# xujiabo/SCREAM

Hardware: AMD Instinct MI355X
Metric: registration pairs/sec (higher is better)
Workload: dtype f32; 1 GPU; BASELINE configs[1]: synthetic 3DMatch_test-like pairs, voxel 0.0625 m, ~5k points/cloud, batch-of-pairs=32 per GPU, A1-A10 per pair (forward 6+6 layers d_model 256, 1-NN thresh 0.1, Kabsch, RE/TE), random-init weights seed 0; lanes=1, steps_in_flight=2, parallelism=dp1 (pairs sharded, metric-row all-gather), rccl_ranks=1, gemm_backend=h2

## Files before the change

### include/scream_hip.h

```cpp
#ifndef SCREAM_HIP_H
#define SCREAM_HIP_H

#include <stdint.h>

#ifdef __cplusplus
extern "C" {
#endif

#define SCREAM_ROW_TILE 128
#define SCREAM_D_MODEL 256
#define SCREAM_NHEAD 8
#define SCREAM_HEAD_DIM 32
#define SCREAM_KV_CHUNK 256

#define SCREAM_EINVAL (-1)
#define SCREAM_EUNSUPPORTED (-2)

enum {
    SCREAM_EPI_NONE = 0,
    SCREAM_EPI_ELU1 = 1,
    SCREAM_EPI_RELU = 2,
    SCREAM_EPI_BIAS_RELU = 3,
    SCREAM_EPI_RES_LN = 4,
    SCREAM_EPI_QKV = 5
// ... 28 lines not shown
                          const float* residual, int64_t ldr, const float* gamma, const float* beta,
                          int32_t layout, int32_t split, int32_t a_exp, int32_t w_exp, void* stream);
int scream_gemm_qkv_split_f32(const float* A, int64_t lda, const void* W_packed, float* Q, int64_t ldq,
                              int64_t M, int32_t N, int32_t K, int32_t n_q, const int32_t* tile_cloud,
                              const int32_t* cloud_row0, const int32_t* cloud_len, int64_t row_base,
                              float* kv_partial, int32_t layout, int32_t split, int32_t a_exp, int32_t w_exp,
                              int32_t k_exp, int32_t v_exp, void* stream);

int64_t scream_proj_image_bytes(int32_t N, int32_t split);
int scream_pack_proj(const float* W, int32_t N, int32_t n_q, int32_t split, int32_t w_exp, void* proj_image, void* stream);
int scream_proj_qkv_f32(const float* x, const void* proj_image, float* Q, int64_t M, int32_t N, int32_t n_q,
                        const int32_t* tile_cloud, const int32_t* cloud_row0, const int32_t* cloud_len,
                        int64_t row_base, float* kv_partial, int32_t split, int32_t a_exp, int32_t w_exp, int32_t k_exp,
                        int32_t v_exp, void* stream);

typedef struct {
    int32_t e_att, e_wm, e_m1, e_w1, e_h, e_w2;
    int32_t e_y, e_wq;
    int32_t e_q;
} scream_tail_exps_t;
int64_t scream_tail_image_bytes(int32_t split, int32_t with_next_q);
int64_t scream_kv_image_bytes(void);
int scream_pack_tail(const float* Wm, const float* W1, const float* W2, const float* Wq_next, int32_t split,
                     const scream_tail_exps_t* exps, void* tail_image, void* stream);
int scream_kv_finalize_image(const float* kv_partial, const int32_t* cloud_row0, const int32_t* cloud_len,
                          int64_t row_base, int32_t cloud_begin, int32_t n_kv, void* kv_image, int32_t n_layers,
                          int64_t partial_layer_stride, int64_t image_layer_stride, int32_t split, void* stream);
int scream_layer_tail_f32(const float* Q, const void* kv_image, const int32_t* tile_cloud,
                          int32_t kv_cloud_offset, const int32_t* cloud_len, const float* x,
                          const void* tail_image, const float* g1, const float* b1, const float* g2,
                          const float* b2, float* y, float* q_next, int64_t M, int32_t split,
                          const scream_tail_exps_t* exps, void* stream);

int scream_pe_embed_ln(const float* xyz, const int32_t* tile_cloud, const float* center,
                       const float* dim_t, const float* emb_w, const float* emb_b,
                       const float* gamma, const float* beta, float* feats, int64_t rows,
                       void* stream);
int scream_pe_embed_ln_frag(const float* xyz, const int32_t* tile_cloud, const float* center,
                            const float* dim_t, const float* emb_w, const float* emb_b,
                            const float* gamma, const float* beta, float* feats, int64_t rows,
                            void* stream);

int scream_kv_reduce(const float* Kf, const float* Vf, int64_t ld, int64_t row_base,
                     const int32_t* cloud_row0, const int32_t* cloud_len, int32_t cloud_begin,
                     int32_t n_kv, int32_t max_chunks, float* partial, float* kv_out, void* stream);

int scream_attn_apply(const float* Qf, int64_t ldq, const float* kv, const int32_t* tile_cloud,
                      int32_t kv_cloud_offset, const int32_t* cloud_len, float* out, int64_t ldo,
                      int64_t rows, void* stream);

int scream_coor_head(const float* X, const float* W, const float* b, float* out, int64_t rows,
                     void* stream);

typedef struct {
    const float* wqkv;
    const float* wq;
    const float* wkv;
    const float* wm;
    const float* w1;
    const float* w2;
    const float* g1; const float* b1;
    const float* g2; const float* b2;
    const void* tail;
    int32_t e_xq, e_xkv, e_wqkv, e_wq, e_wkv, e_wm_g, e_w1_g, e_w2_g;
    int32_t e_k, e_v;
    scream_tail_exps_t tail_exps;
    int32_t tail_next_q;
    const void* proj;
} scream_layer_t;

typedef struct {
    int32_t n_self;
    int32_t n_cross;
    const float* dim_t;
    const float* emb_w; const float* emb_b;
    const float* pre_g; const float* pre_b;
    const scream_layer_t* layers_host;
    const float* c0_w; const float* c0_b;
    const float* c2_w; const float* c2_b;
    const float* c4_w; const float* c4_b;
    const scream_layer_t* stem_tgt_layers_host;
    int32_t gemm_split;
    int32_t e_c0x, e_c0w, e_c2x, e_c2w;
    const float* wkv_cross;
    int32_t e_wkv_cross, e_k_cross, e_v_cross;
    const void* proj_cross;
} scream_model_t;

typedef struct {
    int32_t n_pairs;
    int64_t rows_src;
    int64_t rows_total;
    int32_t max_chunks;
    const float* xyz;
    const float* center;
    const int32_t* tile_cloud;
    const int32_t* cloud_row0;
    const int32_t* cloud_len;
} scream_batch_t;

int64_t scream_forward_workspace_bytes(int64_t rows_src, int64_t rows_total, int32_t n_pairs,
                                       int32_t max_chunks, int32_t fused_tail, int32_t n_cross_batched);

int scream_forward(const scream_model_t* model, const scream_batch_t* batch, void* workspace,
                   int64_t workspace_bytes, float* src_pred, float* feats_out, void* trace,
                   void* stream);

void* scream_trace_create(int32_t capacity);
void scream_trace_destroy(void* trace);
int scream_trace_reset(void* trace);
int scream_trace_read(void* trace, int32_t max_records, float* ms, int32_t* kind, int64_t* m,
                      int32_t* n, int32_t* k);
int scream_trace_read_starts(void* trace, int32_t max_records, float* start_ms);

int scream_nn_search(const float* query, const float* ref, const int32_t* q_row0,
                     const int32_t* q_len, const int32_t* r_row0, const int32_t* r_len,
                     const float* s, int32_t n_pairs, int32_t max_q_len, int32_t max_r_len,
                     int64_t q_rows_total, int64_t r_rows_total, float thresh, float* ref_prep,
                     uint64_t* keys, int32_t* idx, float* dmin, uint8_t* valid, void* stream);

int scream_square_distance(const float* src, const float* dst, float* out, int32_t B, int32_t N,
                           int32_t M, void* stream);

int scream_kabsch_corr(const float* src, const float* ref, const int32_t* src_row0,
                       const int32_t* src_len, const int32_t* ref_row0, const int32_t* idx,
                       const uint8_t* valid, const float* s, const float* c, int32_t n_pairs,
                       float* T_out, int32_t* n_corr, void* stream);

int scream_rigid_transform_3d(const float* A, const float* B, const float* w,
                              float weight_threshold, int32_t bs, int32_t K, float* T_out,
                              void* stream);

int scream_transformation_error(const float* T_pred, const float* T_gt, int32_t n, float* re,
                                float* te, void* stream);

int scream_point_loss(const float* src_pred, const float* src, const int32_t* src_row0, const int32_t* src_len,
                      const float* rot, const float* trans, int32_t n_pairs, float* loss, void* stream);

int64_t scream_icp_workspace_bytes(int64_t src_rows_total, int64_t ref_rows_total, int32_t n_pairs);
// ... 65 lines not shown
```

### scream_amd/_lib.py

```python
from __future__ import annotations

import ctypes as C
import os
from typing import Optional

_HERE = os.path.dirname(os.path.abspath(__file__))
LIB_PATH = os.environ.get("SCREAM_LIB") or os.path.join(_HERE, "libscream_hip.so")
ABI_VERSION = 20

c_f32p = C.POINTER(C.c_float)
c_i32p = C.POINTER(C.c_int32)
c_u8p = C.POINTER(C.c_uint8)
c_u64p = C.POINTER(C.c_uint64)


SPLIT_H1, SPLIT_H2, SPLIT_BF3 = 1, 2, 3


class TailExpsT(C.Structure):
    _fields_ = [(n, C.c_int32) for n in ("e_att", "e_wm", "e_m1", "e_w1", "e_h", "e_w2", "e_y", "e_wq", "e_q")]


class LayerT(C.Structure):
    _fields_ = ([(n, C.c_void_p) for n in ("wqkv", "wq", "wkv", "wm", "w1", "w2", "g1", "b1", "g2", "b2", "tail")] +
                [(n, C.c_int32) for n in ("e_xq", "e_xkv", "e_wqkv", "e_wq", "e_wkv", "e_wm_g", "e_w1_g", "e_w2_g", "e_k", "e_v")] +
                [("tail_exps", TailExpsT), ("tail_next_q", C.c_int32), ("proj", C.c_void_p)])


class ModelT(C.Structure):
    _fields_ = [("n_self", C.c_int32), ("n_cross", C.c_int32), ("dim_t", C.c_void_p), ("emb_w", C.c_void_p),
                ("emb_b", C.c_void_p), ("pre_g", C.c_void_p), ("pre_b", C.c_void_p),
                ("layers_host", C.POINTER(LayerT)), ("c0_w", C.c_void_p), ("c0_b", C.c_void_p),
                ("c2_w", C.c_void_p), ("c2_b", C.c_void_p), ("c4_w", C.c_void_p), ("c4_b", C.c_void_p),
                ("stem_tgt_layers_host", C.POINTER(LayerT)), ("gemm_split", C.c_int32),
                ("e_c0x", C.c_int32), ("e_c0w", C.c_int32), ("e_c2x", C.c_int32), ("e_c2w", C.c_int32),
                ("wkv_cross", C.c_void_p), ("e_wkv_cross", C.c_int32), ("e_k_cross", C.c_int32), ("e_v_cross", C.c_int32),
                ("proj_cross", C.c_void_p)]


class BatchT(C.Structure):
    _fields_ = [("n_pairs", C.c_int32), ("rows_src", C.c_int64), ("rows_total", C.c_int64),
                ("max_chunks", C.c_int32), ("xyz", C.c_void_p), ("center", C.c_void_p),
                ("tile_cloud", C.c_void_p), ("cloud_row0", C.c_void_p), ("cloud_len", C.c_void_p)]


V, I32, I64, F32 = C.c_void_p, C.c_int32, C.c_int64, C.c_float
SIGNATURES = {
    "scream_version": (C.c_char_p, []),
    "scream_abi_version": (C.c_int, []),
    "scream_gemm_f32": (C.c_int, [V, I64, V, V, I64, I64, I32, I32, I32, I32, V, V, I64, V, V, V]),
    "scream_gemm_qkv_f32": (C.c_int, [V, I64, V, V, I64, I64, I32, I32, I32, V, V, V, I64, V, V]),
    "scream_kv_finalize": (C.c_int, [V, V, V, I64, I32, I32, V, V]),
    "scream_pack_w_split": (C.c_int, [V, I32, I32, I32, I32, V, V]),
    "scream_gemm_split_f32": (C.c_int, [V, I64, V, V, I64, I64, I32, I32, I32, I32, V, V, I64, V, V, I32, I32, I32, I32, V]),
    "scream_gemm_qkv_split_f32": (C.c_int, [V, I64, V, V, I64, I64, I32, I32, I32, V, V, V, I64, V, I32, I32, I32, I32, I32, I32, V]),
    "scream_proj_image_bytes": (C.c_int64, [I32, I32]),
    "scream_pack_proj": (C.c_int, [V, I32, I32, I32, I32, V, V]),
    "scream_proj_qkv_f32": (C.c_int, [V, V, V, I64, I32, I32, V, V, V, I64, V, I32, I32, I32, I32, I32, V]),
    "scream_tail_image_bytes": (C.c_int64, [I32, I32]),
    "scream_kv_image_bytes": (C.c_int64, []),
    "scream_pack_tail": (C.c_int, [V, V, V, V, I32, C.POINTER(TailExpsT), V, V]),
    "scream_kv_finalize_image": (C.c_int, [V, V, V, I64, I32, I32, V, I32, I64, I64, I32, V]),
    "scream_layer_tail_f32": (C.c_int, [V, V, V, I32, V, V, V, V, V, V, V, V, V, I64, I32, C.POINTER(TailExpsT), V]),
    "scream_act_layout": (C.c_int, [V, V, I64, I32, V]),
    "scream_pe_embed_ln": (C.c_int, [V, V, V, V, V, V, V, V, V, I64, V]),
    "scream_pe_embed_ln_frag": (C.c_int, [V, V, V, V, V, V, V, V, V, I64, V]),
    "scream_kv_reduce": (C.c_int, [V, V, I64, I64, V, V, I32, I32, I32, V, V, V]),
    "scream_attn_apply": (C.c_int, [V, I64, V, V, I32, V, V, I64, I64, V]),
    "scream_coor_head": (C.c_int, [V, V, V, V, I64, V]),
    "scream_forward_workspace_bytes": (C.c_int64, [I64, I64, I32, I32, I32, I32]),
    "scream_forward": (C.c_int, [C.POINTER(ModelT), C.POINTER(BatchT), V, I64, V, V, V, V]),
    "scream_trace_create": (C.c_void_p, [I32]),
    "scream_trace_destroy": (None, [V]),
    "scream_trace_reset": (C.c_int, [V]),
    "scream_trace_read": (C.c_int, [V, I32, V, V, V, V, V]),
    "scream_trace_read_starts": (C.c_int, [V, I32, V]),
    "scream_nn_search": (C.c_int, [V, V, V, V, V, V, V, I32, I32, I32, I64, I64, F32, V, V, V, V, V, V]),
    "scream_square_distance": (C.c_int, [V, V, V, I32, I32, I32, V]),
    "scream_kabsch_corr": (C.c_int, [V, V, V, V, V, V, V, V, V, I32, V, V, V]),
    "scream_rigid_transform_3d": (C.c_int, [V, V, V, F32, I32, I32, V, V]),
    "scream_transformation_error": (C.c_int, [V, V, I32, V, V, V]),
    "scream_point_loss": (C.c_int, [V, V, V, V, V, V, I32, V, V]),
    "scream_icp_workspace_bytes": (C.c_int64, [I64, I64, I32]),
    "scream_icp_p2p": (C.c_int, [V, V, V, V, V, V, V, V, I32, I32, I32, I64, I64, F32, I32, F32, F32, V, V, V, V, I64, V]),
    "scream_wgrad_workspace_bytes": (C.c_int64, [I64, I32, I32]),
    "scream_gemm_wgrad_f32": (C.c_int, [V, I64, V, I64, I64, I32, I32, V, I32, V, V, I64, V]),
    "scream_wgrad_split_workspace_bytes": (C.c_int64, [I64, I32, I32]),
    "scream_gemm_wgrad_split_f32": (C.c_int, [V, I64, V, I64, I64, I32, I32, V, I32, V, I32, V, I64, V]),
    "scream_ln_fwd": (C.c_int, [V, V, V, V, V, V, V, I64, V]),
    "scream_ln_bwd_workspace_bytes": (C.c_int64, [I64]),
    "scream_ln_bwd": (C.c_int, [V, V, V, V, V, V, V, V, V, V, I32, I64, V, I64, V]),
    "scream_attn_bwd_workspace_bytes": (C.c_int64, [I32, I32]),
    "scream_attn_bwd": (C.c_int, [V, I64, I64, I64, V, V, V, V, I64, I64, I64, V, V, V, V, I32, I32, I32, I32, V, I64, V, V, I64,
                                  V, I64, V]),
    "scream_relu_bwd": (C.c_int, [V, V, I64, V]),
    "scream_add_f32": (C.c_int, [V, V, I64, V]),
    "scream_transpose_f32": (C.c_int, [V, I32, I32, V, V]),
    "scream_coor_head_bwd": (C.c_int, [V, V, V, V, I64, V]),
    "scream_grad3_workspace_bytes": (C.c_int64, [I64]),
    "scream_grad3": (C.c_int, [V, V, V, V, I64, V, I32, V, V, I32, V, I64, V]),
    "scream_pe_embed": (C.c_int, [V, V, V, V, V, V, V, I64, V]),
    "scream_icp_p2p_range": (C.c_int, [V, V, V, V, V, V, V, V, I32, I32, I32, I64, I64, F32, I32, F32, F32, V, V, V, I32, I32, V, V, I64, V]),
    "scream_render_workspace_bytes": (C.c_int64, [I32, I32, I32, I64]),
    "scream_render_depth": (C.c_int, [V, V, V, V, V, V, I32, I32, I32, I64, V, I32, I32, F32, V, V, V, I64, V]),
    "scream_render_depth_bwd": (C.c_int, [V, V, V, I32, I32, I64, V, I32, I32, F32, V, V, V, I64, V, V]),
    "scream_voxel_workspace_bytes": (C.c_int64, [I64, I32]),
    "scream_voxel_down_sample": (C.c_int, [V, V, V, I32, I32, V, V, V, V, V, I64, V]),
}

_lib: Optional[C.CDLL] = None


class ScreamHipError(RuntimeError):
    pass


def load() -> C.CDLL:
    global _lib
    if _lib is not None:
        return _lib
    if os.environ.get("SCREAM_NO_BUILD", "0") != "1" and not os.environ.get("SCREAM_LIB"):
        try:
# ... 30 lines not shown
```

### scream_amd/build.py

```python
from __future__ import annotations

import os
import shutil
import subprocess
import sys
from concurrent.futures import ThreadPoolExecutor

HERE = os.path.dirname(os.path.abspath(__file__))
CSRC = os.path.join(HERE, "csrc")
LIB = os.path.join(HERE, "libscream_hip.so")
ARCH = "gfx950"

SOURCES = {
    "gemm_f32.hip": [],
    "gemm_split.hip": [],
    "proj_ring.hip": ["-mllvm", "-amdgpu-mfma-vgpr-form=1"],
    "tail_split.hip": ["-ffp-contract=off"],
    "embed.hip": [],
    "attention.hip": [],
    "backward.hip": [],
    "forward.hip": [],
    "nn_search.hip": ["-ffp-contract=off"],
    "kabsch.hip": ["-ffp-contract=off"],
    "icp_grid.hip": ["-ffp-contract=off"],
    "render.hip": ["-ffp-contract=off"],
    "voxel.hip": ["-ffp-contract=off"],
}
ASM_LOADS = ("gemm_split.hip", "tail_split.hip", "proj_ring.hip")
NO_SCRATCH = {"proj_ring.hip": ("proj_ring_kernel",), "tail_split.hip": ("tail_kernelINS_7SplitH2", "tail_kernelINS_7SplitH1")}


def _hipcc() -> str:
    exe = shutil.which("hipcc") or "/opt/rocm/bin/hipcc"
    if not os.path.exists(exe):
        raise RuntimeError("hipcc not found: cannot build libscream_hip.so")
    return exe


def _stale() -> bool:
    if not os.path.exists(LIB):
        return True
    t = os.path.getmtime(LIB)
    deps = [os.path.join(CSRC, f) for f in os.listdir(CSRC)] + [os.path.join(HERE, "..", "include", "scream_hip.h"), __file__]
    return any(os.path.getmtime(d) > t for d in deps)


def build(force: bool = False, verbose: bool = False, out: str = None) -> str:
    global LIB
    if out:
        LIB, force = out, True
    if not force and not _stale():
        return LIB
    hipcc = _hipcc()
    objdir = os.path.join(HERE, "build")
    os.makedirs(objdir, exist_ok=True)
    common = [hipcc, "-O3", "-std=c++17", "--offload-arch=" + ARCH, "-fPIC", "-Wall", "-Wno-unused-function"]

    def compile_one(item):
        src, extra = item
        obj = os.path.join(objdir, src.replace(".hip", ".o"))
        cmd = common + extra + ["-c", os.path.join(CSRC, src), "-o", obj]
        r = subprocess.run(cmd, capture_output=True, text=True)
        if r.returncode != 0:
            raise RuntimeError("hipcc failed for %s:\n%s\n%s" % (src, " ".join(cmd), r.stderr))
        if verbose and r.stderr.strip():
            print(r.stderr, file=sys.stderr)
        return obj

    def verify_one(src):
        sys.path.insert(0, os.path.join(HERE, "..", "tools"))
        import asm_inflight_check as chk
        asm = os.path.join(objdir, src.replace(".hip", ".s"))
        cmd = common + SOURCES[src] + ["-S", "--cuda-device-only", os.path.join(CSRC, src), "-o", asm]
        r = subprocess.run(cmd, capture_output=True, text=True)
        if r.returncode != 0:
            raise RuntimeError("hipcc -S failed for %s:\n%s" % (src, r.stderr))
        for name, body in chk.kernels(asm):
            if any(k in name for k in NO_SCRATCH.get(src, ())) and any(("scratch_" in l or "buffer_store" in l) for l in body):
                raise RuntimeError("%s: %s spills registers to scratch (this hipcc allocates registers differently from the one the "
                                   "kernel was written with)" % (src, name))
            bad = chk.check_kernel(name, body)
            if bad:
# ... 33 lines not shown
```

### scream_amd/csrc/forward.hip

```cpp
#include <vector>

#include "common.h"

namespace {

constexpr int D = SCREAM_D_MODEL;
constexpr int KV_ELEMS = (SCREAM_HEAD_DIM + 1) * SCREAM_HEAD_DIM;

struct Workspace {
    float *x0, *x1, *q, *att, *m1, *hid, *kvp, *kv;
    char* kvimg;
    float* kvp_cross;
    char* kvimg_cross;
    int64_t kvp_cross_stride, kvimg_cross_stride;
    int64_t bytes;
};

Workspace carve(void* base, int64_t rows_src, int64_t rows_total, int32_t n_pairs, int32_t max_chunks, bool fused, int32_t n_cross_batched) {
    Workspace w;
    float* p = reinterpret_cast<float*>(base);
    auto take = [&](int64_t n) {
        float* r = p;
        p += (n + 63) / 64 * 64;
        return r;
// ... 234 lines not shown
    SCREAM_REQUIRE(m.layers_host && m.n_self >= 0 && m.n_cross >= 0 &&
                       (m.gemm_split == 0 || m.gemm_split == SCREAM_SPLIT_H1 || m.gemm_split == SCREAM_SPLIT_H2 || m.gemm_split == SCREAM_SPLIT_BF3),
                   SCREAM_EINVAL);
    SCREAM_REQUIRE(b.n_pairs > 0 && b.rows_src > 0 && b.rows_total > b.rows_src && b.max_chunks > 0, SCREAM_EINVAL);
    SCREAM_REQUIRE(b.rows_src % SCREAM_ROW_TILE == 0 && b.rows_total % SCREAM_ROW_TILE == 0, SCREAM_EUNSUPPORTED);
    SCREAM_REQUIRE(b.xyz && b.center && b.tile_cloud && b.cloud_row0 && b.cloud_len, SCREAM_EINVAL);
    int n_layers = m.n_self + 2 * m.n_cross, n_tail = 0;
    for (int i = 0; i < n_layers; ++i) n_tail += m.layers_host[i].tail != nullptr;
    if (m.stem_tgt_layers_host)
        for (int i = 0; i < m.n_self; ++i, ++n_layers) n_tail += m.stem_tgt_layers_host[i].tail != nullptr;
    SCREAM_REQUIRE(n_tail == 0 || (n_tail == n_layers && m.gemm_split != 0), SCREAM_EINVAL);
    uintptr_t base = (reinterpret_cast<uintptr_t>(workspace) + 255) & ~(uintptr_t)255;
    const bool batched_kv = n_tail > 0 && m.wkv_cross != nullptr && m.n_cross > 0;
    const Workspace w = carve(reinterpret_cast<void*>(base), b.rows_src, b.rows_total, b.n_pairs, b.max_chunks, n_tail > 0,
                              batched_kv ? m.n_cross : 0);
    SCREAM_REQUIRE((int64_t)(base - reinterpret_cast<uintptr_t>(workspace)) + w.bytes <= workspace_bytes, SCREAM_EINVAL);
    const Ctx c{stream, reinterpret_cast<Trace*>(trace), m.gemm_split, n_tail > 0};

    const int64_t rs = b.rows_src, ra = b.rows_total;
    {
        Scope sc(c.tr, TR_EMBED, ra, 0, 0, stream);
        if (c.frag)
            TRY(scream_pe_embed_ln_frag(b.xyz, b.tile_cloud, b.center, m.dim_t, m.emb_w, m.emb_b, m.pre_g, m.pre_b, w.x0, ra, stream));
        else
            TRY(scream_pe_embed_ln(b.xyz, b.tile_cloud, b.center, m.dim_t, m.emb_w, m.emb_b, m.pre_g, m.pre_b, w.x0, ra, stream));
    }
    float* cur = w.x0;
    float* nxt = w.x1;
    for (int i = 0; i < m.n_self; ++i) {
        if (!m.stem_tgt_layers_host) {
            TRY(mha_self(c, m.layers_host[i], b, w, cur, nxt, 0, ra, 0, 2 * b.n_pairs));
        } else {
            TRY(mha_self(c, m.layers_host[i], b, w, cur, nxt, 0, rs, 0, b.n_pairs));
            TRY(mha_self(c, m.stem_tgt_layers_host[i], b, w, cur, nxt, rs, ra - rs, b.n_pairs, b.n_pairs));
        }
        float* t = cur;
        cur = nxt;
        nxt = t;
    }
    const float* x_tgt = cur + rs * D;
    if (batched_kv) TRY(cross_kv_all(c, m, b, w, x_tgt));
    for (int i = 0; i < 2 * m.n_cross; ++i) {
        const scream_layer_t& L = m.layers_host[m.n_self + i];
        if (i % 2 == 0) {
            TRY(mha_self(c, L, b, w, cur, nxt, 0, rs, 0, b.n_pairs, c.frag && L.tail_next_q));
        } else {
            const bool q_ready = c.frag && m.layers_host[m.n_self + i - 1].tail_next_q;
            TRY(mha_cross(c, L, b, w, cur, x_tgt, nxt, batched_kv ? w.kvimg_cross + (i / 2) * w.kvimg_cross_stride : nullptr, q_ready));
        }
        float* t = cur;
        cur = nxt;
        nxt = t;
    }
    float* c_mid = c.frag ? w.q : w.m1;
    float* c_out = c.frag ? nxt : w.att;
    TRY(gemm(c, cur, D, m.c0_w, c_mid, D, rs, D, D, SCREAM_EPI_BIAS_RELU, 0, m.c0_b, nullptr, nullptr, nullptr, m.e_c0x, m.e_c0w,
             c.frag ? SCREAM_LAYOUT_A_FRAG : 0));
    TRY(gemm(c, c_mid, D, m.c2_w, c_out, D, rs, D, D, SCREAM_EPI_BIAS_RELU, 0, m.c2_b, nullptr, nullptr, nullptr, m.e_c2x, m.e_c2w));
    {
        Scope sc(c.tr, TR_COOR_HEAD, rs, 0, 0, stream);
        TRY(scream_coor_head(c_out, m.c4_w, m.c4_b, src_pred, rs, stream));
    }
    if (feats_out && c.frag) {
        TRY(scream_act_layout(cur, feats_out, rs, 0, stream));
    } else if (feats_out) {
        hipError_t e = hipMemcpyAsync(feats_out, cur, (size_t)rs * D * sizeof(float), hipMemcpyDeviceToDevice,
                                      as_stream(stream));
        if (e != hipSuccess) return (int)e;
    }
    return 0;
}
```

### scream_amd/model.py

```python
from __future__ import annotations

import ctypes as C
import os
from typing import List, Optional, Sequence, Tuple

import torch
from torch import nn

from . import _lib, ops, scales
from .packing import PackedBatch
from .render import RegistrationRender

D_MODEL = 256
NHEAD = 8


class _MHAParams(nn.Module):

    def __init__(self, d_model: int, nhead: int = NHEAD):
        super().__init__()
        self.q_proj = nn.Linear(d_model, d_model, bias=False)
        self.k_proj = nn.Linear(d_model, d_model, bias=False)
        self.v_proj = nn.Linear(d_model, d_model, bias=False)
        self.merge = nn.Linear(d_model, d_model, bias=False)
# ... 33 lines not shown
            raise NotImplementedError("the gfx950 kernels are built for d_model=256 (8 heads x 32), the only "
                                      "configuration the reference evaluates (evaluate_3d_match.py:188)")
        self.embedding = nn.Conv1d(3, d_model, kernel_size=1, stride=1)
        self.pre_norm = nn.LayerNorm(d_model)
        self.self_layer_num = self_layer_num
        self.cross_layer_num = cross_layer_num
        self.stem = nn.ModuleList([_MHAParams(d_model) for _ in range(self_layer_num)])
        self.cross = nn.ModuleList()
        for _ in range(cross_layer_num):
            self.cross.append(_MHAParams(d_model))
            self.cross.append(_CrossParams(d_model))
        self.coor_mlp = nn.Sequential(nn.Conv1d(d_model, d_model, 1), nn.ReLU(), nn.Conv1d(d_model, d_model, 1),
                                      nn.ReLU(), nn.Conv1d(d_model, 3, 1))
        self.generator = RegistrationRender(rho=24, w=64)
        self._packs = {}
        self._ws = None

    def _layer_modules(self) -> List[_MHAParams]:
        mods = list(self.stem)
        for i, m in enumerate(self.cross):
            mods.append(m if i % 2 == 0 else m.layer)
        return mods

    def _stem_tgt_modules(self) -> Optional[List[_MHAParams]]:
        return None

    gemm_backend = os.environ.get("SCREAM_GEMM", "h2")

    TRAIN_BACKENDS = ("f32", "split")
    _train_backend_default = os.environ.get("SCREAM_TRAIN_GEMM", "f32")

    @classmethod
    def _check_train_backend(cls, value):
        if value not in cls.TRAIN_BACKENDS:
            raise ValueError("train_backend must be one of %s, got %r" % (", ".join(repr(b) for b in cls.TRAIN_BACKENDS), value))
        return value

    @property
    def train_backend(self) -> str:
        return self.__dict__.get("_train_backend", type(self)._train_backend_default)

    @train_backend.setter
    def train_backend(self, value: str) -> None:
        self.__dict__["_train_backend"] = self._check_train_backend(value)

    fused_tail = os.environ.get("SCREAM_FUSED_TAIL", "1") != "0"

    batched_cross_kv = os.environ.get("SCREAM_BATCHED_CROSS_KV", "1") != "0"

    fuse_next_q = os.environ.get("SCREAM_FUSE_NEXT_Q", "1") != "0"

    ring_proj = os.environ.get("SCREAM_RING_PROJ", "1") != "0"

    def _fused_cfg(self, split) -> bool:
        return bool(split and self.fused_tail)

    def _signature(self):
        return (self.fused_tail, self.batched_cross_kv, self.fuse_next_q, self.ring_proj) + tuple((p.data_ptr(), p._version) for p in self.parameters())

    def _layer_inputs(self):
        ln = lambda n: (n.weight, n.bias)
        mods, tgt_mods = self._layer_modules(), self._stem_tgt_modules()
        ns = self.self_layer_num
        pre = ln(self.pre_norm)
        ins, prev = [], pre
        for i in range(ns):
            ins.append((prev, prev))
            prev = ln(mods[i].norm2)
        src_in = prev
        tgt_ins, prev_t = [], pre
        for m in (tgt_mods or []):
            tgt_ins.append((prev_t, prev_t))
            prev_t = ln(m.norm2)
        tgt_in = prev_t if tgt_mods else src_in
        for j in range(2 * self.cross_layer_num):
            ins.append((src_in, src_in if j % 2 == 0 else tgt_in))
            src_in = ln(mods[ns + j].norm2)
        return ins, tgt_ins, src_in

    def _pack_weights(self, backend: Optional[str] = None) -> "_Pack":
        backend = self.gemm_backend if backend is None else backend
        if backend not in ("h2", "x3", "f32", "h1"):
            raise ValueError("gemm_backend must be 'h2', 'x3', 'f32' or 'h1', got %r" % (backend,))
        sig = self._signature()
        if self._packs and next(iter(self._packs.values())).sig != sig:
            torch.cuda.synchronize(self.embedding.weight.device) if self.embedding.weight.is_cuda else None
            self._packs = {}
        pk = self._packs.get(backend)
        if pk is not None:
            return pk
        try:
            pk = self._build_pack(backend, sig)
        except scales.ScaleRangeError as e:
            if backend != "h2":
                raise
            import warnings
            warnings.warn("scream_amd: gemm_backend 'h2' cannot carry these weights (%s); using 'x3' (bf16 x 3 split, scale free, "
                          "same fp32-level accuracy at twice the matrix instructions)" % (e,), RuntimeWarning, stacklevel=3)
            pk = self._pack_weights("x3")
        self._packs[backend] = pk
        return pk

    def _build_pack(self, backend: str, sig) -> "_Pack":
        dev = self.embedding.weight.device
        if dev.type != "cuda":
            raise _lib.ScreamHipError("PointTransformer must be on the MI355X (net.to('cuda:0')) before forward; "
                                      "scream_amd has no CPU path")
        keep = []

        def dev_f32(t):
            t = t.detach().to(device=dev, dtype=torch.float32).contiguous()
# ... 29 lines not shown
            L.wq, L.e_wq = dev_mat(m.q_proj.weight)
            L.wkv, L.e_wkv = dev_mat(wkv)
            ex = scales.layer_exps(m, in_q, in_kv) if fp16_split else {}
            L.e_xq, L.e_xkv, L.e_k, L.e_v = ex.get("e_xq", 0), ex.get("e_xkv", 0), ex.get("e_k", 0), ex.get("e_v", 0)
            wq_next = None
            if id(m) in next_cross:
                nxt = next_cross[id(m)]
                wq_next = mods[nxt].q_proj.weight
                ex.update(e_y=scales.exp_for(scales.ln_bound(*ins[nxt][0])), e_wq=scales.w_exp(wq_next))
            L.tail_exps = ops.tail_exps(**ex)
            L.tail = None
            L.tail_next_q = int(wq_next is not None)
            if split and self.fused_tail:
                f32 = lambda t: t.detach().to(device=dev, dtype=torch.float32)
                img = ops.pack_tail(f32(m.merge.weight), f32(m.mlp[0].weight), f32(m.mlp[2].weight), split, L.tail_exps,
                                    Wq_next=None if wq_next is None else f32(wq_next))
                keep.append(img.data)
                L.tail = img.data_ptr()
                L.wm, L.w1, L.w2 = None, None, None
            else:
                L.wm, L.e_wm_g = dev_mat(m.merge.weight)
                L.w1, L.e_w1_g = dev_mat(m.mlp[0].weight)
                L.w2, L.e_w2_g = dev_mat(m.mlp[2].weight)
            L.g1, L.b1 = dev_f32(m.norm1.weight), dev_f32(m.norm1.bias)
            L.g2, L.b2 = dev_f32(m.norm2.weight), dev_f32(m.norm2.bias)
        mt = _lib.ModelT()
        mt.n_self, mt.n_cross = self.self_layer_num, self.cross_layer_num
        mt.dim_t = dev_f32(pe_dim_t())
        mt.emb_w = dev_f32(self.embedding.weight[:, :, 0])
        mt.emb_b = dev_f32(self.embedding.bias)
        mt.pre_g, mt.pre_b = dev_f32(self.pre_norm.weight), dev_f32(self.pre_norm.bias)
        mt.layers_host = C.cast(layers, C.POINTER(_lib.LayerT))
        mt.stem_tgt_layers_host = C.cast(tgt_layers, C.POINTER(_lib.LayerT)) if tgt_mods else None
        mt.gemm_split = split
        c0w, c2w = self.coor_mlp[0].weight[:, :, 0], self.coor_mlp[2].weight[:, :, 0]
        (mt.c0_w, mt.e_c0w), mt.c0_b = dev_mat(c0w), dev_f32(self.coor_mlp[0].bias)
        (mt.c2_w, mt.e_c2w), mt.c2_b = dev_mat(c2w), dev_f32(self.coor_mlp[2].bias)
        mt.c4_w, mt.c4_b = dev_f32(self.coor_mlp[4].weight[:, :, 0]), dev_f32(self.coor_mlp[4].bias)
        mt.wkv_cross, mt.proj_cross = None, None
        if self._fused_cfg(split) and self.batched_cross_kv and self.cross_layer_num > 0:
            cross = [m for i, m in enumerate(self.cross) if i % 2 == 1]
            stack = torch.cat([torch.cat([c.layer.k_proj.weight[:128], c.layer.v_proj.weight[:128], c.layer.k_proj.weight[128:],
                                          c.layer.v_proj.weight[128:]], dim=0) for c in cross], dim=0)
            mt.wkv_cross, mt.e_wkv_cross = dev_mat(stack)
            if fp16_split and self.ring_proj:
                pp = ops.pack_proj(stack.detach().to(device=dev, dtype=torch.float32), 0, split, mt.e_wkv_cross)
                keep.append(pp.data)
                mt.proj_cross = pp.data_ptr()
            cross_L = [layers[self.self_layer_num + 2 * j + 1] for j in range(self.cross_layer_num)]
            mt.e_k_cross, mt.e_v_cross = min(L.e_k for L in cross_L), min(L.e_v for L in cross_L)
        if fp16_split:
            mt.e_c0x = scales.exp_for(scales.ln_bound(*coor_in))
            mt.e_c2x = scales.exp_for(scales.lin_bound(c0w, *coor_in, bias=self.coor_mlp[0].bias))
        event = torch.cuda.Event()
        event.record(torch.cuda.current_stream(dev))
        return _Pack(backend, sig, mt, (layers, tgt_layers), keep, self._fused_cfg(split), self.cross_layer_num if mt.wkv_cross else 0,
                     event, {torch.cuda.current_stream(dev).cuda_stream})

    def forward_packed(self, batch: PackedBatch, return_feats: bool = False, trace=None, backend: Optional[str] = None):
        pk = self._pack_weights(backend)
        mt = pk.mt
        lib = _lib.load()
        dev = batch.xyz.device
        if ops._stream() not in pk.streams:
            torch.cuda.current_stream(dev).wait_event(pk.event)
            pk.streams.add(ops._stream())
        need = lib.scream_forward_workspace_bytes(batch.rows_src, batch.rows_total, batch.n_pairs, batch.max_chunks, int(pk.fused),
                                                  pk.n_cross_batched)
        if self._ws is None:
            self._ws = {}
        key = (dev, ops._stream())
        ws = self._ws.get(key)
        if ws is None or ws.numel() < need:
            ws = self._ws[key] = torch.empty(need, device=dev, dtype=torch.uint8)
        bt = _lib.BatchT()
        bt.n_pairs, bt.rows_src, bt.rows_total, bt.max_chunks = batch.n_pairs, batch.rows_src, batch.rows_total, batch.max_chunks
        bt.xyz, bt.center = ops._p(batch.xyz), ops._p(batch.center)
        bt.tile_cloud = ops._p(batch.tile_cloud, torch.int32)
        bt.cloud_row0 = ops._p(batch.cloud_row0, torch.int32)
        bt.cloud_len = ops._p(batch.cloud_len, torch.int32)
        src_pred = torch.empty(batch.rows_src, 3, device=dev, dtype=torch.float32)
        feats = torch.empty(batch.rows_src, D_MODEL, device=dev, dtype=torch.float32) if return_feats else None
        _lib.check(lib.scream_forward(C.byref(mt), C.byref(bt), ws.data_ptr(), ws.numel(),
                                      src_pred.data_ptr(), feats.data_ptr() if return_feats else None,
                                      trace, ops._stream()), "scream_forward")
        return (src_pred, feats) if return_feats else src_pred

    def forward_batch(self, srcs: Sequence[torch.Tensor], tgts: Sequence[torch.Tensor],
                      centers: Optional[Sequence[Optional[torch.Tensor]]] = None) -> List[torch.Tensor]:
        batch = PackedBatch.from_pairs(srcs, tgts, centers)
        return [t.clone() for t in batch.unpack_src(self.forward_packed(batch))]

    def train(self, mode: bool = True):
        if mode:
            self._check_train_backend(self.train_backend)
        super().train(mode)
        self._grad_train = bool(mode)
        return self

    def _trains(self) -> bool:
        return getattr(self, "_grad_train", False) and torch.is_grad_enabled()

    def forward_packed_train(self, batch: PackedBatch) -> torch.Tensor:
        if type(self) not in (PointTransformer, DEMTransformer):
            raise NotImplementedError("training is implemented for PointTransformer and DEMTransformer only")
        from . import train as _train
# ... 104 lines not shown
```

### scream_amd/ops.py

```python
from __future__ import annotations

import ctypes as C
import os
from dataclasses import dataclass
from typing import Optional, Tuple

import torch

from . import _lib, scales
from ._lib import SPLIT_BF3, SPLIT_H1, SPLIT_H2, check

EPI_NONE, EPI_ELU1, EPI_RELU, EPI_BIAS_RELU, EPI_RES_LN, EPI_QKV = 0, 1, 2, 3, 4, 5
ROW_TILE = 128
KV_CHUNK = 256
KV_ELEMS = 33 * 32
D_MODEL = 256


def _stream() -> int:
    return torch.cuda.current_stream().cuda_stream


def _p(t: Optional[torch.Tensor], dtype=torch.float32) -> Optional[int]:
    if t is None:
# ... 219 lines not shown
        v_exp = scales.exp_for(amax * float(rl[:, 1].max())) if v_exp is None else v_exp
    check(_lib.load().scream_proj_qkv_f32(_p(x_frag), P.data_ptr(), _p(Q), M, P.N, P.n_q, _p(tile_cloud, torch.int32),
                                          _p(cloud_row0, torch.int32), _p(cloud_len, torch.int32), row_base, _p(part), P.split,
                                          int(a_exp), P.w_exp, int(k_exp), int(v_exp), _stream()), "scream_proj_qkv_f32")
    return Q, part


def kv_finalize(part, cloud_row0, cloud_len, row_base: int, cloud_begin: int, n_kv: int, n_clouds: int) -> torch.Tensor:
    kv = torch.zeros(n_clouds, 8, KV_ELEMS, device=part.device, dtype=torch.float32)
    check(_lib.load().scream_kv_finalize(_p(part), _p(cloud_row0, torch.int32), _p(cloud_len, torch.int32), row_base,
                                         cloud_begin, n_kv, _p(kv), _stream()), "scream_kv_finalize")
    return kv


def pe_embed_ln(xyz, tile_cloud, center, dim_t, emb_w, emb_b, gamma, beta, frag: bool = False) -> torch.Tensor:
    rows = xyz.shape[0]
    feats = torch.empty(rows, D_MODEL, device=xyz.device, dtype=torch.float32)
    lib = _lib.load()
    fn, name = (lib.scream_pe_embed_ln_frag, "scream_pe_embed_ln_frag") if frag else (lib.scream_pe_embed_ln, "scream_pe_embed_ln")
    check(fn(_p(xyz), _p(tile_cloud, torch.int32), _p(center), _p(dim_t), _p(emb_w),
             _p(emb_b), _p(gamma), _p(beta), _p(feats), rows, _stream()), name)
    return feats


def kv_reduce(Kf: torch.Tensor, Vf: torch.Tensor, ld: int, row_base: int, cloud_row0, cloud_len, cloud_begin: int,
              n_kv: int, max_chunks: int, n_clouds: int) -> torch.Tensor:
    dev = Kf.device
    partial = torch.empty(max(n_kv * max_chunks * 8 * KV_ELEMS, 1), device=dev, dtype=torch.float32)
    kv = torch.zeros(n_clouds, 8, KV_ELEMS, device=dev, dtype=torch.float32)
    for t in (Kf, Vf):
        if not t.is_cuda or t.dtype != torch.float32:
            raise TypeError("kv_reduce needs fp32 device tensors")
    check(_lib.load().scream_kv_reduce(Kf.data_ptr(), Vf.data_ptr(), ld, row_base, _p(cloud_row0, torch.int32),
                                       _p(cloud_len, torch.int32), cloud_begin, n_kv, max_chunks, _p(partial),
                                       _p(kv), _stream()), "scream_kv_reduce")
    return kv


def attn_apply(Qf: torch.Tensor, ldq: int, kv, tile_cloud, kv_cloud_offset: int, cloud_len, rows: int) -> torch.Tensor:
    out = torch.empty(rows, D_MODEL, device=kv.device, dtype=torch.float32)
    check(_lib.load().scream_attn_apply(Qf.data_ptr(), ldq, _p(kv), _p(tile_cloud, torch.int32), kv_cloud_offset,
                                        _p(cloud_len, torch.int32), _p(out), D_MODEL, rows, _stream()),
          "scream_attn_apply")
    return out


def coor_head(X: torch.Tensor, W: torch.Tensor, b: torch.Tensor) -> torch.Tensor:
    rows = X.shape[0]
    out = torch.empty(rows, 3, device=X.device, dtype=torch.float32)
    check(_lib.load().scream_coor_head(_p(X), _p(W), _p(b), _p(out), rows, _stream()), "scream_coor_head")
    return out


def nn_search(query: torch.Tensor, ref: torch.Tensor, q_row0, q_len, r_row0, r_len, s: torch.Tensor,
              max_q_len: int, max_r_len: int, thresh: float) -> Tuple[torch.Tensor, torch.Tensor, torch.Tensor]:
    dev = query.device
    qn, rn = query.shape[0], ref.shape[0]
    n_pairs = s.shape[0]
    ref_prep = torch.empty(max(rn, 1), 4, device=dev, dtype=torch.float32)
    keys = torch.empty(max(qn, 1), device=dev, dtype=torch.int64)
    idx = torch.empty(qn, device=dev, dtype=torch.int32)
    dmin = torch.empty(qn, device=dev, dtype=torch.float32)
    valid = torch.empty(qn, device=dev, dtype=torch.uint8)
    check(_lib.load().scream_nn_search(_p(query), _p(ref), _p(q_row0, torch.int32), _p(q_len, torch.int32),
                                       _p(r_row0, torch.int32), _p(r_len, torch.int32), _p(s), n_pairs, max_q_len,
                                       max_r_len, qn, rn, float(thresh), _p(ref_prep), _p(keys, torch.int64),
                                       _p(idx, torch.int32), _p(dmin), _p(valid, torch.uint8), _stream()),
          "scream_nn_search")
    return idx, dmin, valid


def render_workspace(n_pairs: int, n_views: int, w: int, src_rows_total: int, device) -> torch.Tensor:
    need = _lib.load().scream_render_workspace_bytes(n_pairs, n_views, w, src_rows_total)
    if need < 0:
        raise _lib.ScreamHipError("scream_render_workspace_bytes(%d, %d, %d, %d): invalid argument" % (n_pairs, n_views, w, src_rows_total))
    return torch.empty(max(need, 16), device=device, dtype=torch.uint8)


def render_depth(src: torch.Tensor, s_row0, s_len, tgt: torch.Tensor, t_row0, t_len, max_s_len: int, max_t_len: int,
                 rot: torch.Tensor, w: int, rho: float, workspace: Optional[torch.Tensor] = None) -> Tuple[torch.Tensor, torch.Tensor]:
    n_pairs, V = s_row0.shape[0], rot.shape[0]
    dev = src.device
    if workspace is None:
        workspace = render_workspace(n_pairs, V, w, src.shape[0], dev)
    imgs = torch.empty(n_pairs, V, 2, w, w, device=dev, dtype=torch.float32)
    argmax = torch.empty(n_pairs, V, 2, w, w, device=dev, dtype=torch.int32)
    check(_lib.load().scream_render_depth(_p(src), _p(s_row0, torch.int32), _p(s_len, torch.int32), _p(tgt), _p(t_row0, torch.int32),
                                          _p(t_len, torch.int32), n_pairs, int(max_s_len), int(max_t_len), src.shape[0],
                                          _p(rot.reshape(V, 9)), V, int(w), float(rho), _p(imgs), _p(argmax, torch.int32),
                                          _p(workspace, torch.uint8), workspace.numel(), _stream()), "scream_render_depth")
    return imgs, argmax


def render_depth_bwd(dimgs: torch.Tensor, argmax: torch.Tensor, src: torch.Tensor, s_row0, s_len, max_s_len: int,
                     rot: torch.Tensor, w: int, rho: float, workspace: torch.Tensor) -> torch.Tensor:
    n_pairs, V = s_row0.shape[0], rot.shape[0]
    dsrc = torch.zeros(src.shape[0], 3, device=src.device, dtype=torch.float32)
    check(_lib.load().scream_render_depth_bwd(_p(src), _p(s_row0, torch.int32), _p(s_len, torch.int32), n_pairs, int(max_s_len),
                                              src.shape[0], _p(rot.reshape(V, 9)), V, int(w), float(rho), _p(dimgs),
                                              _p(argmax, torch.int32), _p(workspace, torch.uint8), workspace.numel(), _p(dsrc),
                                              _stream()), "scream_render_depth_bwd")
    return dsrc


def voxel_down_sample_packed(xyz: torch.Tensor, row0: torch.Tensor, length: torch.Tensor, max_len: int, voxel: torch.Tensor,
                             want_counts: bool = False) -> Tuple[torch.Tensor, torch.Tensor, Optional[torch.Tensor]]:
# ... 113 lines not shown
```

Measured before the change: 1841 pairs/s.

## Fuse coordinate MLP head into a single ring-pipelined MFMA chain kernel

Adds a persistent kernel that runs the coordinate MLP's two 256x256 bias+ReLU GEMMs and the final 3-wide projection in one pass. Weights are pre-packed into an fp16-split image and streamed through an LDS ring, and the first layer's activations stay in registers as split fragments for the second GEMM. This removes two intermediate activation round-trips to global memory and two kernel launches on the frag/fp16-split path. In exchange it adds a complex hand-scheduled kernel, an extra ABI field in the model struct, and register-pressure risk.

After: 1849 pairs/s, median of 6. Within noise of the previous version (+0.4%).

```diff
diff --git a/include/scream_hip.h b/include/scream_hip.h
--- a/include/scream_hip.h
+++ b/include/scream_hip.h
@@ -104,6 +104,12 @@
 int scream_coor_head(const float* X, const float* W, const float* b, float* out, int64_t rows,
                      void* stream);
 
+int64_t scream_coor_image_bytes(int32_t split);
+int scream_pack_coor(const float* W0, const float* W2, int32_t split, int32_t e_c0w, int32_t e_c2w, void* image, void* stream);
+int scream_coor_chain_f32(const float* x_frag, const void* image, const float* b0, const float* b2, const float* W4,
+                          const float* b4, float* src_pred, int64_t rows, int32_t split, int32_t e_c0x, int32_t e_c0w,
+                          int32_t e_c2x, int32_t e_c2w, void* stream);
+
 typedef struct {
     const float* wqkv;
     const float* wq;
@@ -137,6 +143,7 @@
     const float* wkv_cross;
     int32_t e_wkv_cross, e_k_cross, e_v_cross;
     const void* proj_cross;
+    const void* coor;
 } scream_model_t;
 
 typedef struct {
diff --git a/scream_amd/_lib.py b/scream_amd/_lib.py
--- a/scream_amd/_lib.py
+++ b/scream_amd/_lib.py
@@ -35,7 +35,7 @@
                 ("stem_tgt_layers_host", C.POINTER(LayerT)), ("gemm_split", C.c_int32),
                 ("e_c0x", C.c_int32), ("e_c0w", C.c_int32), ("e_c2x", C.c_int32), ("e_c2w", C.c_int32),
                 ("wkv_cross", C.c_void_p), ("e_wkv_cross", C.c_int32), ("e_k_cross", C.c_int32), ("e_v_cross", C.c_int32),
-                ("proj_cross", C.c_void_p)]
+                ("proj_cross", C.c_void_p), ("coor", C.c_void_p)]
 
 
 class BatchT(C.Structure):
@@ -68,6 +68,9 @@
     "scream_kv_reduce": (C.c_int, [V, V, I64, I64, V, V, I32, I32, I32, V, V, V]),
     "scream_attn_apply": (C.c_int, [V, I64, V, V, I32, V, V, I64, I64, V]),
     "scream_coor_head": (C.c_int, [V, V, V, V, I64, V]),
+    "scream_coor_image_bytes": (C.c_int64, [I32]),
+    "scream_pack_coor": (C.c_int, [V, V, I32, I32, I32, V, V]),
+    "scream_coor_chain_f32": (C.c_int, [V, V, V, V, V, V, V, I64, I32, I32, I32, I32, I32, V]),
     "scream_forward_workspace_bytes": (C.c_int64, [I64, I64, I32, I32, I32, I32]),
     "scream_forward": (C.c_int, [C.POINTER(ModelT), C.POINTER(BatchT), V, I64, V, V, V, V]),
     "scream_trace_create": (C.c_void_p, [I32]),
diff --git a/scream_amd/build.py b/scream_amd/build.py
--- a/scream_amd/build.py
+++ b/scream_amd/build.py
@@ -16,6 +16,7 @@
     "gemm_split.hip": [],
     "proj_ring.hip": ["-mllvm", "-amdgpu-mfma-vgpr-form=1"],
     "tail_split.hip": ["-ffp-contract=off"],
+    "coor_chain.hip": ["-mllvm", "-amdgpu-mfma-vgpr-form=1"],
     "embed.hip": [],
     "attention.hip": [],
     "backward.hip": [],
@@ -26,8 +27,9 @@
     "render.hip": ["-ffp-contract=off"],
     "voxel.hip": ["-ffp-contract=off"],
 }
-ASM_LOADS = ("gemm_split.hip", "tail_split.hip", "proj_ring.hip")
-NO_SCRATCH = {"proj_ring.hip": ("proj_ring_kernel",), "tail_split.hip": ("tail_kernelINS_7SplitH2", "tail_kernelINS_7SplitH1")}
+ASM_LOADS = ("gemm_split.hip", "tail_split.hip", "proj_ring.hip", "coor_chain.hip")
+NO_SCRATCH = {"proj_ring.hip": ("proj_ring_kernel",), "tail_split.hip": ("tail_kernelINS_7SplitH2", "tail_kernelINS_7SplitH1"),
+              "coor_chain.hip": ("coor_chain_kernelINS_7SplitH2", "coor_chain_kernelINS_7SplitH1")}
 
 
 def _hipcc() -> str:
diff --git a/scream_amd/csrc/coor_chain.hip b/scream_amd/csrc/coor_chain.hip
--- /dev/null
+++ b/scream_amd/csrc/coor_chain.hip
@@ -0,0 +1,245 @@
+#include <type_traits>
+
+#include "ring.h"
+
+namespace {
+
+constexpr int C_STAGES = 16;
+constexpr int C_RIDE0 = 2;
+constexpr int C_CONST_FLOATS = 5 * 256 + 16;
+
+struct CoorArgs {
+    const float* x;
+    const char* img;
+    const float *b0, *b2, *w4, *b4;
+    float* out;
+    int n_tiles;
+    float s_x;
+    float c1;
+    float s_h;
+    float c2;
+};
+
+template <class SP>
+__global__ __launch_bounds__(TT, 1) void coor_chain_kernel(CoorArgs ca) {
+    static_assert(SP::SCALED, "built for the fp16 splits");
+    typedef typename SP::vec V;
+    constexpr int NP = SP::NP;
+    constexpr int STAGE = stage_bytes<SP>();
+    constexpr int PIECES = wave_pieces<SP>();
+    constexpr int NV = 12 / SP::NPROD;
+    __shared__ __attribute__((aligned(16))) char smem[T_SLOTS * STAGE + C_CONST_FLOATS * 4];
+    const int tid = threadIdx.x, lane = tid & 63;
+    const int wave = __builtin_amdgcn_readfirstlane(tid >> 6);
+    const int half = lane >> 5;
+    const unsigned v_lane16 = lane * 16;
+    int tile = blockIdx.x;
+    if (tile >= ca.n_tiles) return;
+
+    float* cst = reinterpret_cast<float*>(smem + T_SLOTS * STAGE);
+    cst[tid] = ca.b0[tid];
+    cst[256 + tid] = ca.b2[tid];
+    cst[512 + tid] = ca.w4[tid];
+    cst[768 + tid] = ca.w4[256 + tid];
+    cst[1024 + tid] = ca.w4[512 + tid];
+    if (tid < 3) cst[1280 + tid] = ca.b4[tid];
+    const float* cl = cst + 4 * half;
+
+    auto dma_piece = [&](unsigned qq, int u) __attribute__((always_inline)) {
+        const unsigned src = qq % (unsigned)C_STAGES, slot = qq % (unsigned)T_SLOTS;
+        const char* sbase = ca.img + (size_t)src * STAGE + (wave * PIECES + (u & ~3)) * 1024;
+        dma_1k(sbase + v_lane16, smem + slot * STAGE + (wave * PIECES + (u & ~3)) * 1024, u & 3);
+    };
+    unsigned q = 0;
+#pragma unroll
+    for (int u = 0; u < PIECES; ++u) dma_piece(0, u);
+#pragma unroll
+    for (int u = 0; u < PIECES; ++u) dma_piece(1, u);
+
+    auto rows_of = [&](int t) { return ca.x + ((int64_t)t * 128 + wave * 32) * SCREAM_D_MODEL; };
+    f32x4 raw[8][4];
+#pragma unroll
+    for (int seg = 0; seg < 8; ++seg) ld_asm4<1024, true>(raw[seg], rows_of(tile) + seg * 1024, v_lane16);
+
+    while (tile < ca.n_tiles) {
+        const int tile_next = tile + (int)gridDim.x;
+        const bool has_next = tile_next < ca.n_tiles;
+        const float* x_next = rows_of(has_next ? tile_next : tile);
+        const int seg_step = has_next ? 1024 : 0;
+
+        VM_WAIT(0);
+#pragma unroll
+        for (int seg = 0; seg < 8; ++seg)
+#pragma unroll
+            for (int a = 0; a < 4; ++a) pin(raw[seg][a]);
+        __builtin_amdgcn_sched_barrier(0);
+        V xp[16][NP];
+#pragma unroll
+        for (int seg = 0; seg < 8; ++seg)
+#pragma unroll
+            for (int s2 = 0; s2 < 2; ++s2) {
+                V tmp[NP];
+                split8s<SP>(raw[seg][2 * s2], raw[seg][2 * s2 + 1], ca.s_x, tmp);
+#pragma unroll
+                for (int p = 0; p < NP; ++p) {
+                    asm volatile("" : "+a"(tmp[p]));
+                    xp[2 * seg + s2][p] = tmp[p];
+                }
+            }
+        __builtin_amdgcn_sched_barrier(0);
+
+        V hp[16][NP];
+        V hnew[2][NP];
+        f32x16 acc[2];
+        float o0 = 0.f, o1 = 0.f, o2 = 0.f;
+
+        auto relu = [&](float v) __attribute__((always_inline)) {
+            float r;
+            asm("v_max_f32 %0, 0, %1" : "=v"(r) : "v"(v));
+            return r;
+        };
+        auto ride1 = [&](const f32x16& t, int cc, int k) __attribute__((always_inline)) {
+            const int s2 = k >> 2, j = (2 * k) & 7;
+            const int f = 32 * cc + 8 * (k >> 1) + 2 * (k & 1);
+            const float x0 = relu(__builtin_fmaf(t[2 * k], ca.c1, cl[f]));
+            const float x1 = relu(__builtin_fmaf(t[2 * k + 1], ca.c1, cl[f + 1]));
+            SP::split2s(x0, x1, ca.s_h, j, hnew[s2]);
+            if ((k & 3) == 3) {
+#pragma unroll
+                for (int p = 0; p < NP; ++p) {
+                    asm volatile("" : "+a"(hnew[s2][p]));
+                    hp[2 * cc + s2][p] = hnew[s2][p];
+                }
+            }
+        };
+        auto ride2 = [&](const f32x16& t, int cc, int k) __attribute__((always_inline)) {
+            const int f = 32 * cc + 8 * (k >> 1) + 2 * (k & 1);
+#pragma unroll
+            for (int e = 0; e < 2; ++e) {
+                const float h = relu(__builtin_fmaf(t[2 * k + e], ca.c2, cl[256 + f + e]));
+                o0 = __builtin_fmaf(h, cl[512 + f + e], o0);
+                o1 = __builtin_fmaf(h, cl[768 + f + e], o1);
+                o2 = __builtin_fmaf(h, cl[1024 + f + e], o2);
+            }
+        };
+
+        auto stage = [&](auto ss) __attribute__((always_inline)) {
+            constexpr int s = decltype(ss)::value;
+            if (s == 0) ring_barrier<0>(); else ring_barrier<PIECES>();
+            __builtin_amdgcn_sched_barrier(0);
+            if (s >= 8) ld_asm4<1024, true>(raw[s & 7], x_next + (s & 7) * seg_step, v_lane16);
+            __builtin_amdgcn_sched_barrier(0);
+            const char* wb = smem + (q % T_SLOTS) * STAGE + lane * 16;
+            V wf[T_PF][NP];
+#pragma unroll
+            for (int g0 = 0; g0 < T_PF - 1; ++g0)
+#pragma unroll
+                for (int p = 0; p < NP; ++p) wf[g0][p] = ld_frag<V>(wb + (p * 16 + g0) * 1024);
+#pragma unroll
+            for (int g = 0; g < 16; ++g) {
+                if (g + T_PF - 1 < 16) {
+#pragma unroll
+                    for (int p = 0; p < NP; ++p) wf[(g + T_PF - 1) % T_PF][p] = ld_frag<V>(wb + (p * 16 + g + T_PF - 1) * 1024);
+                }
+                if (g < PIECES) dma_piece(q + 2, g);
+                if (s > 0 && g >= C_RIDE0 && g < C_RIDE0 + 8) {
+                    if (s <= 8) ride1(acc[(s + 1) & 1], (s + 7) & 7, g - C_RIDE0);
+                    else ride2(acc[(s + 1) & 1], (s + 7) & 7, g - C_RIDE0);
+                }
+                mfma_group<SP, NV>(acc[s & 1], wf[g % T_PF], s < 8 ? xp[g] : hp[g], g == 0);
+            }
+            ++q;
+        };
+#define ST(n) stage(std::integral_constant<int, n>{})
+        ST(0); ST(1); ST(2); ST(3); ST(4); ST(5); ST(6); ST(7);
+        ST(8); ST(9); ST(10); ST(11); ST(12); ST(13); ST(14); ST(15);
+#undef ST
+        __builtin_amdgcn_sched_barrier(0);
+#pragma unroll
+        for (int k = 0; k < 8; ++k) ride2(acc[1], 7, k);
+        o0 += __shfl_xor(o0, 32);
+        o1 += __shfl_xor(o1, 32);
+        o2 += __shfl_xor(o2, 32);
+        if (half == 0) {
+            float* op = ca.out + ((int64_t)tile * 128 + wave * 32 + lane) * 3;
+            op[0] = o0 + cst[1280];
+            op[1] = o1 + cst[1281];
+            op[2] = o2 + cst[1282];
+        }
+        __builtin_amdgcn_sched_barrier(0);
+        tile = tile_next;
+    }
+    VM_WAIT(0);
+}
+
+template <class SP>
+__global__ void pack_coor_kernel(const float* __restrict__ W0, const float* __restrict__ W2, float s_w0, float s_w2,
+                                 typename SP::vec* __restrict__ out) {
+    const int t = blockIdx.x * blockDim.x + threadIdx.x;
+    if (t >= C_STAGES * 16 * 64) return;
+    const int lane = t & 63, frag = (t >> 6) & 15, stage = t >> 10;
+    const int m = lane & 31, half = lane >> 5;
+    const float* W = stage < 8 ? W0 : W2;
+    const float s = stage < 8 ? s_w0 : s_w2;
+    typename SP::vec p[SP::NP];
+#pragma unroll
+    for (int j = 0; j < 8; ++j)
+        SP::split1(W[(int64_t)(32 * (stage & 7) + m) * 256 + 32 * (frag >> 1) + chunk_k(frag & 1, half, j)] * s, j, p);
+#pragma unroll
+    for (int pl = 0; pl < SP::NP; ++pl) out[(((int64_t)stage * SP::NP + pl) * 16 + frag) * 64 + lane] = p[pl];
+}
+
+bool coor_split_ok(int32_t split) { return split == SCREAM_SPLIT_H2 || split == SCREAM_SPLIT_H1; }
+bool coor_exp_ok(int e) { return e >= -60 && e <= 60; }
+
+}
+
+extern "C" int64_t scream_coor_image_bytes(int32_t split) {
+    if (!coor_split_ok(split)) return SCREAM_EINVAL;
+    return (int64_t)C_STAGES * split * 16 * 1024;
+}
+
+extern "C" int scream_pack_coor(const float* W0, const float* W2, int32_t split, int32_t e_c0w, int32_t e_c2w, void* image, void* stream) {
+    SCREAM_REQUIRE(W0 && W2 && image && coor_split_ok(split), SCREAM_EINVAL);
+    SCREAM_REQUIRE(coor_exp_ok(e_c0w) && coor_exp_ok(e_c2w) && (reinterpret_cast<uintptr_t>(image) & 15) == 0, SCREAM_EINVAL);
+    const dim3 grid(C_STAGES * 16 * 64 / 256), block(256);
+    if (split == SCREAM_SPLIT_H2)
+        pack_coor_kernel<SplitH2><<<grid, block, 0, as_stream(stream)>>>(W0, W2, exp2i(e_c0w), exp2i(e_c2w), reinterpret_cast<f16x8*>(image));
+    else
+        pack_coor_kernel<SplitH1><<<grid, block, 0, as_stream(stream)>>>(W0, W2, exp2i(e_c0w), exp2i(e_c2w), reinterpret_cast<f16x8*>(image));
+    SCREAM_LAUNCH_CHECK();
+    return 0;
+}
+
+extern "C" int scream_coor_chain_f32(const float* x_frag, const void* image, const float* b0, const float* b2, const float* W4,
+                                     const float* b4, float* src_pred, int64_t rows, int32_t split, int32_t e_c0x, int32_t e_c0w,
+                                     int32_t e_c2x, int32_t e_c2w, void* stream) {
+    SCREAM_REQUIRE(x_frag && image && b0 && b2 && W4 && b4 && src_pred && coor_split_ok(split), SCREAM_EINVAL);
+    SCREAM_REQUIRE(rows >= 0 && rows % SCREAM_ROW_TILE == 0, SCREAM_EUNSUPPORTED);
+    SCREAM_REQUIRE(coor_exp_ok(e_c0x) && coor_exp_ok(e_c0w) && coor_exp_ok(e_c2x) && coor_exp_ok(e_c2w), SCREAM_EINVAL);
+    SCREAM_REQUIRE(((reinterpret_cast<uintptr_t>(x_frag) | reinterpret_cast<uintptr_t>(image)) & 15) == 0 &&
+                       ((reinterpret_cast<uintptr_t>(b0) | reinterpret_cast<uintptr_t>(b2) | reinterpret_cast<uintptr_t>(W4) |
+                         reinterpret_cast<uintptr_t>(b4) | reinterpret_cast<uintptr_t>(src_pred)) & 3) == 0,
+                   SCREAM_EINVAL);
+    const int64_t tiles = rows / SCREAM_ROW_TILE;
+    if (tiles == 0) return 0;
+    SCREAM_REQUIRE(tiles < (1ll << 31), SCREAM_EUNSUPPORTED);
+    CoorArgs ca;
+    ca.x = x_frag;
+    ca.img = reinterpret_cast<const char*>(image);
+    ca.b0 = b0;
+    ca.b2 = b2;
+    ca.w4 = W4;
+    ca.b4 = b4;
+    ca.out = src_pred;
+    ca.n_tiles = (int)tiles;
+    ca.s_x = exp2i(e_c0x);
+    ca.c1 = exp2i(-e_c0x - e_c0w);
+    ca.s_h = exp2i(e_c2x);
+    ca.c2 = exp2i(-e_c2x - e_c2w);
+    const unsigned grid = tiles < T_MAX_GRID ? (unsigned)tiles : (unsigned)T_MAX_GRID;
+    if (split == SCREAM_SPLIT_H2) coor_chain_kernel<SplitH2><<<dim3(grid), dim3(TT), 0, as_stream(stream)>>>(ca);
+    else coor_chain_kernel<SplitH1><<<dim3(grid), dim3(TT), 0, as_stream(stream)>>>(ca);
+    SCREAM_LAUNCH_CHECK();
+    return 0;
+}
diff --git a/scream_amd/csrc/forward.hip b/scream_amd/csrc/forward.hip
--- a/scream_amd/csrc/forward.hip
+++ b/scream_amd/csrc/forward.hip
@@ -310,12 +310,15 @@
         cur = nxt;
         nxt = t;
     }
-    float* c_mid = c.frag ? w.q : w.m1;
-    float* c_out = c.frag ? nxt : w.att;
-    TRY(gemm(c, cur, D, m.c0_w, c_mid, D, rs, D, D, SCREAM_EPI_BIAS_RELU, 0, m.c0_b, nullptr, nullptr, nullptr, m.e_c0x, m.e_c0w,
-             c.frag ? SCREAM_LAYOUT_A_FRAG : 0));
-    TRY(gemm(c, c_mid, D, m.c2_w, c_out, D, rs, D, D, SCREAM_EPI_BIAS_RELU, 0, m.c2_b, nullptr, nullptr, nullptr, m.e_c2x, m.e_c2w));
-    {
+    if (c.frag && m.coor && (c.split == SCREAM_SPLIT_H2 || c.split == SCREAM_SPLIT_H1)) {
+        Scope sc(c.tr, SCREAM_EPI_BIAS_RELU, rs, 2 * D, D, stream);
+        TRY(scream_coor_chain_f32(cur, m.coor, m.c0_b, m.c2_b, m.c4_w, m.c4_b, src_pred, rs, c.split, m.e_c0x, m.e_c0w, m.e_c2x, m.e_c2w, stream));
+    } else {
+        float* c_mid = c.frag ? w.q : w.m1;
+        float* c_out = c.frag ? nxt : w.att;
+        TRY(gemm(c, cur, D, m.c0_w, c_mid, D, rs, D, D, SCREAM_EPI_BIAS_RELU, 0, m.c0_b, nullptr, nullptr, nullptr, m.e_c0x, m.e_c0w,
+                 c.frag ? SCREAM_LAYOUT_A_FRAG : 0));
+        TRY(gemm(c, c_mid, D, m.c2_w, c_out, D, rs, D, D, SCREAM_EPI_BIAS_RELU, 0, m.c2_b, nullptr, nullptr, nullptr, m.e_c2x, m.e_c2w));
         Scope sc(c.tr, TR_COOR_HEAD, rs, 0, 0, stream);
         TRY(scream_coor_head(c_out, m.c4_w, m.c4_b, src_pred, rs, stream));
     }
diff --git a/scream_amd/model.py b/scream_amd/model.py
--- a/scream_amd/model.py
+++ b/scream_amd/model.py
@@ -109,11 +109,13 @@
 
     ring_proj = os.environ.get("SCREAM_RING_PROJ", "1") != "0"
 
+    coor_chain = os.environ.get("SCREAM_COOR_CHAIN", "1") != "0"
+
     def _fused_cfg(self, split) -> bool:
         return bool(split and self.fused_tail)
 
     def _signature(self):
-        return (self.fused_tail, self.batched_cross_kv, self.fuse_next_q, self.ring_proj) + tuple((p.data_ptr(), p._version) for p in self.parameters())
+        return (self.fused_tail, self.batched_cross_kv, self.fuse_next_q, self.ring_proj, self.coor_chain) + tuple((p.data_ptr(), p._version) for p in self.parameters())
 
     def _layer_inputs(self):
         ln = lambda n: (n.weight, n.bias)
@@ -249,6 +251,12 @@
         if fp16_split:
             mt.e_c0x = scales.exp_for(scales.ln_bound(*coor_in))
             mt.e_c2x = scales.exp_for(scales.lin_bound(c0w, *coor_in, bias=self.coor_mlp[0].bias))
+        mt.coor = None
+        if fp16_split and self.fused_tail and self.coor_chain:
+            f32 = lambda t: t.detach().to(device=dev, dtype=torch.float32)
+            pc = ops.pack_coor(f32(c0w), f32(c2w), split, mt.e_c0w, mt.e_c2w)
+            keep.append(pc.data)
+            mt.coor = pc.data_ptr()
         event = torch.cuda.Event()
         event.record(torch.cuda.current_stream(dev))
         return _Pack(backend, sig, mt, (layers, tgt_layers), keep, self._fused_cfg(split), self.cross_layer_num if mt.wkv_cross else 0,
diff --git a/scream_amd/ops.py b/scream_amd/ops.py
--- a/scream_amd/ops.py
+++ b/scream_amd/ops.py
@@ -295,6 +295,44 @@
     return out
 
 
+@dataclass
+class PackedCoor:
+    data: torch.Tensor
+    split: int
+    e_c0w: int
+    e_c2w: int
+
+    def data_ptr(self) -> int:
+        return self.data.data_ptr()
+
+
+def pack_coor(W0: torch.Tensor, W2: torch.Tensor, split: Optional[int] = None, e_c0w: Optional[int] = None,
+              e_c2w: Optional[int] = None) -> PackedCoor:
+    split = SPLIT_H2 if split is None else split
+    W0, W2 = (w.detach().to(torch.float32).contiguous() for w in (W0, W2))
+    assert W0.shape == (D_MODEL, D_MODEL) and W2.shape == (D_MODEL, D_MODEL)
+    e_c0w = scales.w_exp(W0) if e_c0w is None else int(e_c0w)
+    e_c2w = scales.w_exp(W2) if e_c2w is None else int(e_c2w)
+    lib = _lib.load()
+    nbytes = lib.scream_coor_image_bytes(split)
+    if nbytes <= 0:
+        raise _lib.ScreamHipError("scream_coor_image_bytes(%d) = %d (the coordinate chain needs an fp16 split)" % (split, nbytes))
+    out = torch.empty(nbytes, device=W0.device, dtype=torch.uint8)
+    check(lib.scream_pack_coor(_p(W0), _p(W2), split, e_c0w, e_c2w, _p(out, torch.uint8), _stream()), "scream_pack_coor")
+    return PackedCoor(out, split, e_c0w, e_c2w)
+
+
+def coor_chain(x_frag: torch.Tensor, P: PackedCoor, b0: torch.Tensor, b2: torch.Tensor, W4: torch.Tensor, b4: torch.Tensor,
+               e_c0x: int, e_c2x: int, out: Optional[torch.Tensor] = None) -> torch.Tensor:
+    rows = x_frag.shape[0]
+    assert x_frag.shape[1] == D_MODEL and W4.shape == (3, D_MODEL)
+    if out is None:
+        out = torch.empty(rows, 3, device=x_frag.device, dtype=torch.float32)
+    check(_lib.load().scream_coor_chain_f32(_p(x_frag), P.data_ptr(), _p(b0), _p(b2), _p(W4), _p(b4), _p(out), rows, P.split,
+                                            int(e_c0x), P.e_c0w, int(e_c2x), P.e_c2w, _stream()), "scream_coor_chain_f32")
+    return out
+
+
 def nn_search(query: torch.Tensor, ref: torch.Tensor, q_row0, q_len, r_row0, r_len, s: torch.Tensor,
               max_q_len: int, max_r_len: int, thresh: float) -> Tuple[torch.Tensor, torch.Tensor, torch.Tensor]:
     dev = query.device
```
